# PASSIONLab/BELLA

Hardware: AMD Instinct MI355X
Metric: candidate overlap pairs/sec (higher is better)
Workload: dtype u16/u32 integer

## Files before the change

### bella_amd/csrc/bella_hip.hip

```cpp
#include <hip/hip_runtime.h>
#include <hipcub/hipcub.hpp>

#include <algorithm>
#include <cmath>
#include <initializer_list>
#include <iterator>
#include <map>
#include <cstdarg>
#include <cstdio>
#include <cstdlib>
#include <chrono>
#include <cstring>
#include <string>
#include <thread>
#include <vector>

#include "../../include/bella_hip.h"
#include "assemble.hpp"
#include "comm.hpp"
#include "core.hpp"
#include "fastq.hpp"
#include "kcount.hpp"
#include "logan.hpp"
#include "order.hpp"
// ... 80 lines not shown
    __host__ __device__ uint32_t operator()(const uint8_t& v) const { return (uint32_t)v; }
};
struct CountU64 {
    __host__ __device__ uint64_t operator()(const uint32_t& v) const { return (uint64_t)(v & ~kOrderedBit); }
};

}

struct bella_ctx {
    int device = 0;
    hipStream_t stream = nullptr;
    std::string err;
    uint32_t debug = 0;

    uint32_t nreads = 0;
    uint64_t total_bases = 0;
    Buf packed, roff;
    uint32_t nkmers = 0, kmer_size = 0;
    uint64_t nnz = 0;
    bool have_reads = false, have_matrix = false, have_pairs = false, have_alns = false;
    std::vector<std::string> names;
    std::vector<uint32_t> host_lens;
    bool have_tuples = false;
    uint64_t kc_ntuples = 0;
    uint32_t kc_nkmers = 0, kc_k = 0;
    uint32_t kc_bfirst = 0, kc_brows = 0;
    Buf kc_nk, kc_koff, kc_hist, kc_keys, kc_alt, kc_runlen, kc_flag, kc_slot, kc_nruns, kc_dcode, kc_dcount, kc_hkey, kc_hval, kc_found,
        kc_tstart, kc_cursor, kc_sel, kc_ringo, kc_ringp, kc_opos, kc_oid, kc_opos2, kc_oid2;
    Buf Bptr, Bk, Bpos, Bent, rowF, Aent, Aent2, Aov, Arow, Bloc;
    bool have_rowlists = false;
    bool want_rowlists = false;
    uint32_t part_first = 0, part_stride = 1;
    uint32_t layout_first = 0, layout_stride = 1;
    uint64_t owned_nnz = 0;
    uint64_t live_nnz = 0;
    uint64_t sym_sig[6] = {};
    uint64_t layout_gen = 0;
    uint32_t range_lo = 0, range_hi = 0xFFFFFFFFu;
    bool have_panel = false;
    uint32_t panel_first = 0, panel_rows = 0;
    uint64_t panel_nnz = 0;
    Buf t_kmer, t_read, t_pos, tstart, Bk_tmp, Bpos_tmp, rowcnt, asm_ws, asm_cls;
    Buf lk_key, lk_key2, lk_val, lk_val2, w, wscan, lk_rinfo;
    uint64_t flops = 0, npairs = 0;
    uint32_t pair_ratio1024 = 1024;
    bool long_list_sample = false;
#ifdef BELLA_DEV_PROF
    Buf prof;
#endif
    Buf flopsr, flopptr, nnzC, colptrC, rowlists, tiercaps, tmp_pairs, tmp_ext, pairs, ext, sortscr, ws,
        status, cubtmp, plist_hv, overflow, ctl, retry, orderlist, order_ws;
    bool order_attr = false;
    Buf w_f, w_off, w_key, w_key2, w_idx, w_idx2, w_hv, w_ovfl, w_plist, w_scr, w_rlen, w_rstart, w_rrank, w_redo, w_segfirst,
        w_toff, w_table, w_nruns, w_desc, w_gtab, w_gcount, w_gbase, w_rfirst, w_aent2, w_aov;
    uint32_t n_wide = 0;
    uint32_t n_retry = 0;
    uint32_t n_overflow = 0;
    uint64_t nalns = 0;
    Buf alns, seeds, xest, xest2, xids, xorder, xres, xstate, xlive, lg_res, lg_redo, lg_scratch;
    bool have_traces = false;
    std::vector<bella_trace> traces;
    std::vector<uint32_t> trace_ops;
    std::vector<uint32_t> batch_ops;
    bool have_batch_ops = false;
    bella_trace_stats trace_stats{};
    Buf tr_exts, tr_lists, tr_res, tr_pres, tr_opoff, tr_dirs, tr_scr, tr_ops;
    bella_timings tm{};
    hipEvent_t ev[12]{};
    uint32_t* pinned = nullptr;
    Stager stager;
    bella_ingest_stats ingest{};
    int caps_state = 0;
    ncclComm_t comm = nullptr;
    const Rccl* api = nullptr;
    int comm_ranks = 0, comm_rank = 0;
    Buf comm_meta;
    bool pass_known = false;
    uint64_t pass_sig[6] = {};
    uint32_t pass_tcnt[20] = {};
    uint64_t pass_products = 0;
    uint64_t pass_wide_products[2] = {};
    bool pass_rare_free = false;
    bool pass_big_free = false;
    uint32_t tier_caps[kNumTiers] = {};
    uint32_t ntiers = 0;
    bool tiers_from_env = false;
    uint64_t kcount_budget = 1ull << 30, wide_budget = 1ull << 30;
    bool lane_order_ok = true;
    uint64_t xdrop_class_min = 4ull * 4096 * 64;
    BufPool pool;
    uint32_t layout_inline = 0;
    uint32_t tune_layout_order = 0;
    uint32_t tune_inline = 0;
    uint32_t tune_row_path = 0;
    uint32_t tune_compact_b = 0;
    uint32_t tune_dist_layout = 2;
    bool dist_agreed = false;
    bool layout_dist = false;
    uint64_t tune_cache_bytes = 192ull << 20;
    uint32_t xdrop_variant = 1;
    size_t lds_attr[24] = {};
    hipStream_t side[kNumTiers + 1]{};
    hipEvent_t fork = nullptr, join[kNumTiers + 1]{};
};

namespace {

int fail(bella_ctx* c, int code, const char* fmt, ...) {
    char b[512];
    va_list ap;
    va_start(ap, fmt);
    vsnprintf(b, sizeof(b), fmt, ap);
    va_end(ap);
    if (c) c->err = b;
    return code;
}

#define HIPCHK(c, call)                                                                                           \
    do {                                                                                                          \
        hipError_t e_ = (call);                                                                                   \
        if (e_ != hipSuccess)                                                                                     \
            return fail(c, BELLA_ERR_HIP, "%s failed: %s (%s:%d)", #call, hipGetErrorString(e_), __FILE__, __LINE__); \
    } while (0)
#define KCHK(c) HIPCHK(c, hipGetLastError())
#define NCCLCHK(c, call)                                                                                          \
    do {                                                                                                          \
        ncclResult_t r_ = (call);                                                                                 \
        if (r_ != ncclSuccess)                                                                                    \
            return fail(c, BELLA_ERR_HIP, "%s failed: %s", #call, c->api && c->api->GetErrorString ? c->api->GetErrorString(r_) : "RCCL error"); \
    } while (0)

void release(Buf& b);
void trim_pool(BufPool& pl) {
    for (auto& q : pl.free) (void)hipFree(q.first);
    pl.free.clear();
    pl.bytes = 0;
}
int ensure_bytes(bella_ctx* c, Buf& b, size_t bytes) {
    if (bytes == 0) bytes = 16;
    if (b.cap >= bytes) return 0;
    release(b);
    BufPool& pl = c->pool;
    b.pool = &pl;
    const size_t want = bytes + bytes / 16 + 256;
    int best = -1;
    for (int i = 0; i < (int)pl.free.size(); ++i)
        if (pl.free[i].second >= want && pl.free[i].second <= 2 * want + (64ull << 20) && (best < 0 || pl.free[i].second < pl.free[best].second)) best = i;
    if (best >= 0) {
        b.p = pl.free[best].first; b.cap = pl.free[best].second;
        pl.bytes -= b.cap;
        pl.free.erase(pl.free.begin() + best);
        return 0;
    }
    if (pl.arena.base) {
        void* q = pl.arena.take(want);
        if (q) { b.p = q; b.cap = Arena::round(want); return 0; }
    }
    hipError_t e = hipMalloc(&b.p, want);
    if (e != hipSuccess && !pl.free.empty()) {
        (void)hipGetLastError();
        trim_pool(pl);
        e = hipMalloc(&b.p, want);
    }
    if (e != hipSuccess) {
        b.p = nullptr;
        return fail(c, BELLA_ERR_NOMEM, "hipMalloc(%zu) failed: %s", want, hipGetErrorString(e));
// ... 292 lines not shown
    uint32_t st = 0;
    int rc = read_status(c, &st);
    if (rc) return rc;
    rc = status_to_error(c, st);
    if (rc) return rc;
    c->pair_ratio1024 = ratio1024;
    release(c->lk_key); release(c->lk_key2); release(c->lk_val); release(c->lk_val2); release(c->w); release(c->wscan); release(c->lk_rinfo);
    c->tm.layout_ms = ev_ms(c->ev[4], c->ev[5]);
    c->have_matrix = true;
    c->layout_gen++;
    c->have_pairs = c->have_alns = false;
    return 0;
}

int check_params(bella_ctx* c, const bella_params* p) {
    if (!p) return fail(c, BELLA_ERR_BAD_ARG, "params is NULL");
    if (p->kmer_size != c->kmer_size)
        return fail(c, BELLA_ERR_BAD_ARG, "params.kmer_size (%u) differs from the matrix's (%u)", p->kmer_size, c->kmer_size);
    if (!p->skip_alignment) {
        if (p->xdrop > 127) return fail(c, BELLA_ERR_BAD_ARG, "params.xdrop must fit Xavier's int8 scores (<= 127)");
        if (!(p->error_rate >= 0.0 && p->error_rate <= 1.0) || !(p->delta_chernoff >= 0.0 && p->delta_chernoff <= 1.0))
            return fail(c, BELLA_ERR_BAD_ARG, "params.error_rate and params.delta_chernoff must lie in [0, 1]");
    }
    return 0;
}

}

extern "C" {

int bella_hip_abi_version(void) { return BELLA_HIP_ABI_VERSION; }

int bella_hip_device_count(void) {
    int n = 0;
    if (hipGetDeviceCount(&n) != hipSuccess) return 0;
    return n;
}

const char* bella_hip_strerror(int code) {
    switch (code) {
        case BELLA_OK: return "ok";
        case BELLA_ERR_NO_DEVICE: return "no gfx950 HIP device";
        case BELLA_ERR_HIP: return "HIP runtime error";
        case BELLA_ERR_BAD_ARG: return "bad argument";
        case BELLA_ERR_BAD_BASE: return "read contains a character other than ACGT";
        case BELLA_ERR_READ_TOO_LONG: return "read too long for 16-bit positions";
        case BELLA_ERR_TUPLE_ORDER: return "tuples not grouped by read";
        case BELLA_ERR_STATE: return "call order violated";
        case BELLA_ERR_ROW_TOO_LARGE: return "output column too large";
        case BELLA_ERR_BINS: return "more than 16 overlap bins";
        case BELLA_ERR_NOMEM: return "out of device memory";
    }
    return "unknown error";
}

const char* bella_hip_last_error(const bella_ctx* ctx) { return ctx ? ctx->err.c_str() : "null context"; }

int bella_hip_init(int device, bella_ctx** out) {
    if (!out) return BELLA_ERR_BAD_ARG;
    *out = nullptr;
    int n = 0;
    if (hipGetDeviceCount(&n) != hipSuccess || n <= 0 || device < 0 || device >= n) return BELLA_ERR_NO_DEVICE;
    hipDeviceProp_t prop;
    if (hipGetDeviceProperties(&prop, device) != hipSuccess) return BELLA_ERR_NO_DEVICE;
    if (std::strncmp(prop.gcnArchName, "gfx950", 6) != 0) return BELLA_ERR_NO_DEVICE;
    bella_ctx* c = new bella_ctx();
    c->device = device;
    c->ntiers = 0;
    for (uint32_t t = 0; t < kNumTiers; ++t) { c->tier_caps[t] = kTierCapsDefault[t]; c->ntiers = t + 1; if (kTierCapsDefault[t] == 65535) break; }
    hipError_t he = hipSetDevice(device);
    if (he == hipSuccess) he = hipStreamCreate(&c->stream);
    for (auto& e : c->ev) if (he == hipSuccess) he = hipEventCreate(&e);
    {
        int least = 0, greatest = 0;
        if (he == hipSuccess) he = hipDeviceGetStreamPriorityRange(&least, &greatest);
        int si = 0;
        for (auto& st : c->side) {
            if (he == hipSuccess) he = hipStreamCreateWithPriority(&st, hipStreamNonBlocking, si < 2 || si == kNumTiers ? greatest : least);
            ++si;
        }
    }
    if (he == hipSuccess) he = hipEventCreateWithFlags(&c->fork, hipEventDisableTiming);
    for (auto& e : c->join) if (he == hipSuccess) he = hipEventCreateWithFlags(&e, hipEventDisableTiming);
    if (he != hipSuccess) { bella_hip_destroy(c); return BELLA_ERR_HIP; }
    if (hipHostMalloc((void**)&c->pinned, 512, hipHostMallocDefault) != hipSuccess) { delete c; return BELLA_ERR_NOMEM; }
    if (ensure_bytes(c, c->status, 256)) { delete c; return BELLA_ERR_NOMEM; }
    (void)hipMemset(c->status.p, 0, 256);
    {
        uint32_t bad = 1;
        k_lane_order_selftest<<<1, 64, 0, c->stream>>>(ptr<uint32_t>(c->status) + 12);
        if (hipMemcpyAsync(&bad, ptr<uint32_t>(c->status) + 12, 4, hipMemcpyDeviceToHost, c->stream) != hipSuccess ||
            hipStreamSynchronize(c->stream) != hipSuccess) bad = 1;
        c->lane_order_ok = bad == 0;
        c->tm.lane_order = c->lane_order_ok ? 1u : 2u;
    }
    *out = c;
    return 0;
}

void bella_hip_destroy(bella_ctx* c) {
    if (!c) return;
    (void)hipSetDevice(c->device);
    (void)hipStreamSynchronize(c->stream);
    if (c->comm && c->api) { (void)c->api->CommDestroy(c->comm); c->comm = nullptr; }
    release(c->comm_meta);
    Buf* all[] = {&c->packed, &c->roff, &c->Bptr, &c->Bk, &c->Bpos, &c->Bent, &c->rowF, &c->Aent, &c->Aent2, &c->Aov, &c->Arow, &c->Bloc, &c->t_kmer, &c->t_read, &c->t_pos,
                  &c->tstart, &c->Bk_tmp, &c->Bpos_tmp, &c->rowcnt, &c->asm_ws, &c->asm_cls, &c->lk_key, &c->lk_key2, &c->lk_val, &c->lk_val2, &c->lk_rinfo,
                  &c->w, &c->wscan, &c->flopsr, &c->flopptr, &c->nnzC, &c->colptrC,
                  &c->rowlists, &c->tiercaps, &c->tmp_pairs, &c->tmp_ext, &c->pairs, &c->ext, &c->sortscr, &c->ws,
                  &c->status, &c->cubtmp, &c->alns, &c->seeds, &c->plist_hv, &c->overflow, &c->ctl, &c->retry, &c->orderlist, &c->order_ws, &c->w_f, &c->w_off, &c->w_key, &c->w_key2, &c->w_idx, &c->w_idx2, &c->w_hv, &c->w_ovfl,
                  &c->w_plist, &c->w_scr, &c->w_rlen, &c->w_rstart, &c->w_rrank, &c->w_redo, &c->w_segfirst, &c->w_toff, &c->w_table, &c->w_nruns, &c->w_desc, &c->w_gtab, &c->w_gcount, &c->w_gbase, &c->w_rfirst, &c->w_aent2, &c->w_aov, &c->kc_nk, &c->kc_koff, &c->kc_hist, &c->kc_keys, &c->kc_alt, &c->kc_runlen,
                  &c->kc_flag, &c->kc_slot, &c->kc_nruns, &c->kc_dcode, &c->kc_dcount, &c->kc_hkey, &c->kc_hval, &c->kc_found, &c->kc_tstart, &c->kc_cursor, &c->kc_sel, &c->kc_ringo, &c->kc_ringp, &c->kc_opos, &c->kc_oid, &c->kc_opos2, &c->kc_oid2, &c->xest, &c->xest2, &c->xids, &c->xorder, &c->xres, &c->xstate, &c->xlive, &c->lg_res, &c->lg_redo, &c->lg_scratch};
    for (Buf* b : all) release(*b);
    trim_pool(c->pool);
    if (c->pool.arena.base) { (void)hipFree(c->pool.arena.base); c->pool.arena = Arena(); }
    for (auto& e : c->ev) (void)hipEventDestroy(e);
    for (auto& st : c->side) (void)hipStreamDestroy(st);
    (void)hipEventDestroy(c->fork);
    for (auto& e : c->join) (void)hipEventDestroy(e);
    (void)hipStreamDestroy(c->stream);
    if (c->pinned) (void)hipHostFree(c->pinned);
    c->stager.destroy();
    delete c;
}

int bella_hip_set_tuning(bella_ctx* c, uint32_t what, const uint64_t* values, uint32_t n) {
    if (!c || (n && !values)) return BELLA_ERR_BAD_ARG;
    switch (what) {
        case BELLA_TUNE_LDS_TIERS: {
            uint32_t caps[kNumTiers];
            uint32_t m = 0;
            for (uint32_t q = 0; q < n && m + 1 < kNumTiers; ++q) {
                const uint64_t v = values[q];
                if (v < 64 || v > 11008 || (m && v <= caps[m - 1])) return fail(c, BELLA_ERR_BAD_ARG, "tier caps must ascend within [64, 11008]");
                caps[m++] = (uint32_t)v;
            }
            if (m) {
                for (uint32_t t = 0; t < m; ++t) c->tier_caps[t] = caps[t];
                c->tier_caps[m] = 65535;
                c->ntiers = m + 1;
                c->tiers_from_env = true;
            } else {
                c->ntiers = 0;
                for (uint32_t t = 0; t < kNumTiers; ++t) { c->tier_caps[t] = kTierCapsDefault[t]; c->ntiers = t + 1; if (kTierCapsDefault[t] == 65535) break; }
                c->tiers_from_env = false;
            }
            c->caps_state = 0;
            c->pass_known = false;
            return 0;
        }
        case BELLA_TUNE_KCOUNT_BUDGET: c->kcount_budget = n && values[0] ? values[0] : (1ull << 30); return 0;
        case BELLA_TUNE_WIDE_BUDGET: c->wide_budget = n && values[0] ? values[0] : (1ull << 30); return 0;
        case BELLA_TUNE_XDROP_VARIANT:
            if (n && values[0] > 3) return fail(c, BELLA_ERR_BAD_ARG, "x-drop variant 0..3");
            c->xdrop_variant = n ? (uint32_t)values[0] : 1u;
            return 0;
        case BELLA_TUNE_XDROP_CLASS_MIN: c->xdrop_class_min = n ? values[0] : 4ull * 4096 * 64; return 0;
        case BELLA_TUNE_ROW_LISTS:
            if (n && values[0] > 1) return fail(c, BELLA_ERR_BAD_ARG, "row lists: 0 or 1");
            c->want_rowlists = n && values[0] == 1;
            return 0;
        case BELLA_TUNE_LAYOUT_ORDER:
            if (n && values[0] > 1) return fail(c, BELLA_ERR_BAD_ARG, "layout order: 0 (k-mer order) or 1 (first appearance)");
            c->tune_layout_order = n ? (uint32_t)values[0] : 0u;
            return 0;
        case BELLA_TUNE_INLINE_ENTRIES:
// ... 1885 lines not shown
        if (main_l >= 0) { rc = side_stream(2); if (rc) return rc; sst = c->side[2]; }
        a.rowdesc = ptr<uint4>(c->rowlists) + (size_t)(g_ntiers - 1) * nr;
        a.nrows = tcnt[g_ntiers - 1];
        a.cap = tier_caps[g_ntiers - 1];
        a.dcap = a.cap;
        const unsigned grid = a.nrows < kGlobalGrid ? a.nrows : kGlobalGrid;
        if (c->have_rowlists) k_spgemm_rows_global<true><<<grid, kGlobalBlock, 0, sst>>>(a);
        else k_spgemm_rows_global<false><<<grid, kGlobalBlock, 0, sst>>>(a);
        KCHK(c);
        launches++;
    }
    {
        int side_left = 3 - nwhole - (global_tier ? 1 : 0);
        for (int l = nl - 1; l >= 0; --l) {
            if (!ln[l].rows || (whole_cu(l) && l != main_l)) continue;
            int later = 0;
            for (int m2 = 0; m2 < l; ++m2) later += ln[m2].rows ? 1 : 0;
            const bool on_main = l == main_l || side_left == 0 || later == 0;
            if (!on_main) side_left--;
            rc = launch_class(l, on_main);
            if (rc) return rc;
        }
    }
    if (c->n_wide) {
        hipStream_t const main_stream = c->stream, wst = c->side[kNumTiers];
        c->stream = wst;
        int rw = 0;
        if (wide_begun) rw = wide_batch_finish(c, wide_batch, false);
        else {
            HIPCHK(c, hipStreamWaitEvent(wst, c->ev[3], 0));
            rw = wide_columns();
            if (!rw) rw = run_wide(c, a, c->n_wide, widelist, wide_products);
        }
        c->stream = main_stream;
        if (rw) { (void)hipStreamSynchronize(wst); return rw; }
        HIPCHK(c, hipEventRecord(c->join[kNumTiers], wst));
        HIPCHK(c, hipStreamWaitEvent(c->stream, c->join[kNumTiers], 0));
    }
    for (int w = 0; w < 3; ++w)
        if (used[w]) {
            HIPCHK(c, hipEventRecord(c->join[w], c->side[w]));
            HIPCHK(c, hipStreamWaitEvent(c->stream, c->join[w], 0));
        }
    FoldArgs fa;
    fa.ctl = a.ctl;
    fa.overflow = a.overflow;
    fa.flopptr = a.flopptr;
    fa.plist = a.plist;
    fa.roff = a.roff;
    fa.packed = a.packed;
    fa.tmp_pairs = a.tmp_pairs;
    fa.tmp_ext = a.tmp_ext;
    fa.sort_scratch = ptr<uint16_t>(c->sortscr);
    fa.k = a.k;
    fa.binSize = a.binSize;
    auto rerun_columns = [&]() -> int {
        a.rowlist = ptr<uint32_t>(c->retry);
        a.rowdesc = nullptr;
        a.nrows_dev = ptr<uint32_t>(c->ctl) + kCtlRetry;
        if (c->have_rowlists) k_spgemm_rows_global<true><<<kRerunGrid, kGlobalBlock, 0, c->stream>>>(a);
        else k_spgemm_rows_global<false><<<kRerunGrid, kGlobalBlock, 0, c->stream>>>(a);
        KCHK(c);
        return 0;
    };
    auto finish = [&]() -> int {
        if ((uint64_t)nr + 1 <= kScanSingleMax) {
            k_scan_counts<<<1, 1024, 0, c->stream>>>(ptr<uint32_t>(c->nnzC), ptr<uint64_t>(c->colptrC), nr + 1);
            KCHK(c);
        } else {
            hipcub::TransformInputIterator<uint64_t, CountU64, const uint32_t*> it(ptr<uint32_t>(c->nnzC), CountU64());
            size_t tb = c->cubtmp.cap;
            HIPCHK(c, hipcub::DeviceScan::ExclusiveSum(c->cubtmp.p, tb, it, ptr<uint64_t>(c->colptrC), (int)nr + 1, c->stream));
        }
        EVREC(6);
        if (nr) {
            OrderArgs oa;
            oa.flopptr = ptr<uint64_t>(c->flopptr); oa.colptrC = ptr<uint64_t>(c->colptrC); oa.nnzC = ptr<uint32_t>(c->nnzC);
            oa.flops = ptr<uint32_t>(c->flopsr);
            oa.nreads = nr; oa.i0 = i0; oa.stride = c->part_stride; oa.nown = nown;
            oa.tmp_pairs = ptr<bella_pair>(c->tmp_pairs); oa.tmp_ext = want_ext ? ptr<bella_pair_ext>(c->tmp_ext) : nullptr;
            oa.pairs = ptr<bella_pair>(c->pairs); oa.ext = want_ext ? ptr<bella_pair_ext>(c->ext) : nullptr;
            oa.totals = (uint64_t*)(d_ctl + kCtlTotals);
            oa.nbig = d_ctl + kCtlOrderBig; oa.biglist = ptr<uint32_t>(c->orderlist); oa.ws = ptr<uint8_t>(c->order_ws);
            if (nown <= kOrderOneLaunchMax) {
                k_order_wave<kOrderWaveHt, 0><<<nblk(nown ? nown : 1, kOrderBlock / 64), kOrderBlock, 0, c->stream>>>(oa);
                KCHK(c);
            } else {
                k_order_wave<512, 0><<<nblk(nown ? nown : 1, kOrderBlock / 64), kOrderBlock, 0, c->stream>>>(oa);
                KCHK(c);
                k_order_wave<kOrderWaveHt, 512><<<nblk(nown ? nown : 1, kOrderBlock / 64), kOrderBlock, 0, c->stream>>>(oa);
                KCHK(c);
            }
            if (!skip_big) {
                k_order_block<<<kOrderBigGrid, kOrderBlock, (size_t)6 * kOrderLdsHt, c->stream>>>(oa);
                KCHK(c);
            }
        }
        EVREC(7);
        HIPCHK(c, hipMemcpyAsync(ctl_host, d_ctl, 4 * kCtlWords, hipMemcpyDeviceToHost, c->stream));
        return 0;
    };
    if (!skip_rare) { rc = rerun_columns(); if (rc) return rc; }
    EVREC(5);
    if (!skip_rare) { k_fold_overflow<<<256, 64, 0, c->stream>>>(fa); KCHK(c); EVREC(8); }
    return finish();
    };
#undef EVREC
    rc = enqueue();
    if (rc) return rc;
    HIPCHK(c, hipStreamSynchronize(c->stream));
    if ((skip_rare && (ctl_host[kCtlRetry] || ctl_host[kCtlOverflow])) || (skip_big && ctl_host[kCtlOrderBig])) {
        c->pass_rare_free = false;
        c->pass_big_free = false;
        if (depth > 0) return fail(c, BELLA_ERR_STATE, "internal: rare kernels still skipped");
        return run_spgemm(c, p, status_out, depth + 1);
    }
    const uint32_t* const tcnt = c->pass_tcnt;
    const uint64_t Fub = c->pass_products;
    uint64_t P = 0, F = 0;
    std::memcpy(&P, ctl_host + kCtlTotals, 8);
    std::memcpy(&F, ctl_host + kCtlTotals + 2, 8);
    rc = status_to_error(c, ctl_host[kCtlStatus] & ~1u);
    if (rc) return rc;
    *status_out = ctl_host[kCtlStatus];
    c->n_overflow = ctl_host[kCtlOverflow];
    c->n_retry = ctl_host[kCtlRetry];
    c->npairs = P;
    c->flops = F;
    if (F != Fub || std::memcmp(ctl_host + kCtlTierCnt, tcnt, 4 * (g_ntiers + 1)) != 0) {
        c->pass_known = false;
        return fail(c, BELLA_ERR_STATE, "internal: product total %llu / tier lengths differ from the ones the pass was sized with (%llu)",
                    (unsigned long long)F, (unsigned long long)Fub);
    }
    c->pass_known = true;
    c->pass_rare_free = c->n_retry == 0 && c->n_overflow == 0 && c->n_wide == 0;
    c->pass_big_free = ctl_host[kCtlOrderBig] == 0;
    c->tm.symbolic_ms = ev_ms(c->ev[2], c->ev[3]);
    c->tm.spgemm_ms = ev_ms(c->ev[3], c->ev[5]);
    c->tm.fold_ms = skip_rare ? 0.f : ev_ms(c->ev[5], c->ev[8]);
    c->tm.compact_ms = ev_ms(c->ev[6], c->ev[7]);
    c->tm.overlap_total_ms = ev_ms(c->ev[2], c->ev[7]);
    c->tm.spgemm_launches = launches;
    c->tm.retry_columns = c->n_retry;
    c->tm.overflow_pairs = c->n_overflow;
#ifdef BELLA_DEV_PROF
    {
        unsigned long long ph[10 * kNumTiers];
        HIPCHK(c, hipMemcpy(ph, c->prof.p, sizeof(ph), hipMemcpyDeviceToHost));
        static const char* nm[9] = {"expand", "gather+insert", "count-scan", "scatter+singles", "rank/overlay", "parents", "walks", "emit", "head (descriptor + first entries + table init)"};
        for (int l = 0; l < nl; ++l) {
            const unsigned long long* q = ph + 10 * l;
            if (!q[9]) continue;
            double tot = 1e-9;
            for (int n = 0; n < 9; ++n) tot += (double)q[n];
            fprintf(stderr, "[bella_hip prof] class cap %u (%llu columns, %.0f cycles each):", tier_caps[ln[l].hi], q[9], tot / (double)q[9]);
            for (int n = 0; n < 9; ++n) fprintf(stderr, " %s %.1f%%", nm[n], 100.0 * (double)q[n] / tot);
            fprintf(stderr, "\n");
        }
    }
#endif
    return 0;
}

static uint32_t owned_columns(const bella_ctx* c, uint32_t* i0_out) {
    const uint32_t nr = c->nreads;
    const uint32_t hi = c->range_hi < nr ? c->range_hi : nr;
    uint32_t i0 = c->range_lo + (c->part_first + c->part_stride - c->range_lo % c->part_stride) % c->part_stride;
    const uint32_t nown = i0 < hi ? (hi - i0 + c->part_stride - 1) / c->part_stride : 0;
    if (!nown) i0 = 0;
    if (i0_out) *i0_out = i0;
    return nown;
}

int bella_hip_overlap(bella_ctx* c, const bella_params* p, uint64_t* npairs, uint64_t* flops) {
    if (!c) return BELLA_ERR_BAD_ARG;
// ... 778 lines not shown
```

### bella_amd/csrc/order.hpp

```cpp
#pragma once
#include <hip/hip_runtime.h>
#include <stdint.h>
#include "../../include/bella_hip.h"
#include "core.hpp"
#include "slotorder.hpp"
#include "util.hpp"

namespace bella {

constexpr uint32_t kOrderWaveHt = 1024;
constexpr uint32_t kOrderLdsHt = 16384;
constexpr uint32_t kOrderBlock = 256;
constexpr uint32_t kOrderBigGrid = 512;
constexpr uint32_t kOrderOneLaunchMax = 32768;
constexpr uint64_t kOrderWsBytes = (uint64_t)6 * 65536;

struct OrderArgs {
    const uint64_t* flopptr;
    const uint64_t* colptrC;
    const uint32_t* nnzC;
    const uint32_t* flops;
    uint32_t nreads, i0, stride, nown;
    const bella_pair* tmp_pairs;
    const bella_pair_ext* tmp_ext;
    bella_pair* pairs;
    bella_pair_ext* ext;
    uint64_t* totals;
    uint32_t* nbig;
    uint32_t* biglist;
    uint8_t* ws;
};

__device__ __forceinline__ void order_copy_record(const OrderArgs& a, uint64_t from, uint64_t to, uint32_t cid) {
    uint4 rec = *(const uint4*)(a.tmp_pairs + from);
    asm volatile("" : "+v"(rec.y));
    rec.y = cid;
    *(uint4*)(a.pairs + to) = rec;
    if (a.ext) a.ext[to] = a.tmp_ext[from];
}

__device__ __forceinline__ bool wave_next_free(const uint32_t* T2, uint16_t* nf, uint32_t ht) {
    const uint32_t lane = lane_id();
    const uint32_t nb = (ht + 63u) >> 6;
    uint32_t carry = 0xFFFFFFFFu;
#pragma unroll 1
    for (int sweep = 0; sweep < 2; ++sweep) {
        for (uint32_t b = nb; b-- > 0;) {
            const uint32_t s = (b << 6) + lane;
            const bool empty = s < ht && T2[s] == kEmpty;
            const unsigned long long m = __ballot(empty);
            if (sweep == 1 && s < ht) {
                const unsigned long long up = m >> lane;
                nf[s] = (uint16_t)(up ? s + (uint32_t)__ffsll((long long)up) - 1u : carry);
            }
            if (m) carry = (b << 6) + (uint32_t)__ffsll((long long)m) - 1u;
        }
        if (carry == 0xFFFFFFFFu) return false;
    }
    return true;
}
__device__ __forceinline__ void wave_rank_slots(const uint32_t* T2, uint16_t* ord, uint32_t ht) {
    const uint32_t lane = lane_id();
    const uint32_t nb = (ht + 63u) >> 6;
    uint32_t base = 0;
    for (uint32_t b = 0; b < nb; ++b) {
        const uint32_t s = (b << 6) + lane;
        const uint32_t it = s < ht ? T2[s] : kEmpty;
        const unsigned long long m = __ballot(it != kEmpty);
        if (it != kEmpty) ord[base + (uint32_t)__popcll(m & ((1ull << lane) - 1ull))] = (uint16_t)(it & 0xFFFFu);
        base += (uint32_t)__popcll(m);
    }
}

template <uint32_t HT, uint32_t HTLO>
__global__ __launch_bounds__(kOrderBlock) void k_order_wave(OrderArgs a) {
    __shared__ uint32_t s_T2[kOrderBlock / 64][HT];
    __shared__ uint16_t s_ord[kOrderBlock / 64][HT];
    const uint32_t j0 = blockIdx.x * (kOrderBlock / 64) + wave_id();
    const uint32_t lane = lane_id();
    if (HTLO == 0 && j0 == 0 && lane == 0) a.totals[0] = a.colptrC[a.nreads];
    if (j0 >= a.nown) return;
    const uint32_t i = a.i0 + j0 * a.stride;
    uint32_t nz = a.nnzC[i];
    uint64_t src = a.flopptr[i], dst = a.colptrC[i];
    uint32_t tmax = a.flops[i];
    asm volatile("" : "+v"(nz), "+v"(src), "+v"(dst), "+v"(tmax));
    const uint32_t d = nz & ~kOrderedBit;
    if (!d) return;
    if (nz & kOrderedBit) {
        if (HTLO == 0) for (uint32_t r = lane; r < d; r += 64) order_copy_record(a, src + r, dst + r, i);
        return;
    }
    const uint32_t ht = pow2_at_least(16u, d);
    if (ht > kOrderWaveHt) {
        if (HTLO == 0 && lane == 0) a.biglist[atomicAdd(a.nbig, 1u)] = i;
        return;
    }
    if (ht > HT || ht <= HTLO) return;
    uint32_t* T2 = s_T2[wave_id()];
    uint16_t* ord = s_ord[wave_id()];
    for (uint32_t s = lane; s < ht; s += 64) T2[s] = kEmpty;
    constexpr uint32_t NI = HT / 64;
    uint32_t key[NI], fp[NI];
#pragma unroll
    for (uint32_t u = 0; u < NI; ++u) {
        const uint32_t j = lane + 64 * u;
        key[u] = 0; fp[u] = 0xFFFFFFFFu;
        if (j < d) { const uint2 kf = *(const uint2*)(a.tmp_pairs + src + j); key[u] = kf.x; fp[u] = kf.y; }
    }
    group_sync<64>();
    uint32_t prev = 0;
    for (uint32_t rd = 0;; ++rd) {
        const uint32_t bound = round_bound(rd, ht, d, tmax);
        if (rd) { (void)wave_next_free(T2, ord, ht); group_sync<64>(); }
#pragma unroll
        for (uint32_t u = 0; u < NI; ++u) {
            if (fp[u] < prev || fp[u] >= bound) continue;
            const uint32_t home = (key[u] * 107u) & (ht - 1), item = (fp[u] << 16) | (lane + 64 * u);
            if (rd) slot_insert<true>(T2, ord, ht - 1, home, item);
            else slot_insert<false>(T2, ord, ht - 1, home, item);
        }
        group_sync<64>();
        if (bound >= tmax) break;
        prev = bound;
    }
    wave_rank_slots(T2, ord, ht);
    group_sync<64>();
    {
        uint32_t r = lane;
        for (; r + 192 < d; r += 256) {
            uint4 rec[4];
#pragma unroll
            for (uint32_t u = 0; u < 4; ++u) rec[u] = *(const uint4*)(a.tmp_pairs + src + ord[r + 64 * u]);
#pragma unroll
            for (uint32_t u = 0; u < 4; ++u) { asm volatile("" : "+v"(rec[u].y)); rec[u].y = i; *(uint4*)(a.pairs + dst + r + 64 * u) = rec[u]; }
            if (a.ext) {
#pragma unroll
                for (uint32_t u = 0; u < 4; ++u) a.ext[dst + r + 64 * u] = a.tmp_ext[src + ord[r + 64 * u]];
            }
        }
        for (; r < d; r += 64) order_copy_record(a, src + ord[r], dst + r, i);
    }
}

__global__ __launch_bounds__(kOrderBlock) void k_order_block(OrderArgs a) {
    extern __shared__ __attribute__((aligned(16))) uint8_t smem[];
    __shared__ uint32_t scr[16];
    const uint32_t nbig = *a.nbig;
    const uint32_t tid = threadIdx.x;
    for (uint32_t x = blockIdx.x; x < nbig; x += gridDim.x) {
        const uint32_t i = a.biglist[x];
        const uint32_t d = a.nnzC[i] & ~kOrderedBit;
        const uint64_t src = a.flopptr[i], dst = a.colptrC[i];
        const uint32_t ht = pow2_at_least(16u, d);
        uint32_t* T2;
        uint16_t* ord;
        if (ht <= kOrderLdsHt) { T2 = (uint32_t*)smem; ord = (uint16_t*)(smem + (size_t)4 * kOrderLdsHt); }
        else { uint8_t* w = a.ws + (uint64_t)blockIdx.x * kOrderWsBytes; T2 = (uint32_t*)w; ord = (uint16_t*)(w + (size_t)4 * 65536); }
        for (uint32_t s = tid; s < ht; s += kOrderBlock) T2[s] = kEmpty;
        __syncthreads();
        const uint32_t tmax = a.flops[i];
        uint32_t prev = 0;
        for (uint32_t rd = 0;; ++rd) {
            const uint32_t bound = round_bound(rd, ht, d, tmax);
            if (rd) { (void)build_next_free<(int)kOrderBlock>(T2, ord, ht, scr); __syncthreads(); }
            for (uint32_t j = tid; j < d; j += kOrderBlock) {
                const uint2 kf = *(const uint2*)(a.tmp_pairs + src + j);
                if (kf.y < prev || kf.y >= bound) continue;
                const uint32_t home = (kf.x * 107u) & (ht - 1), item = (kf.y << 16) | j;
                if (rd) slot_insert<true>(T2, ord, ht - 1, home, item);
                else slot_insert<false>(T2, ord, ht - 1, home, item);
            }
            __syncthreads();
            if (bound >= tmax) break;
            prev = bound;
        }
        {
            const uint32_t c = (ht + kOrderBlock - 1) / kOrderBlock;
            const uint32_t lo = tid * c < ht ? tid * c : ht, hi = lo + c < ht ? lo + c : ht;
            uint32_t occ = 0;
            for (uint32_t s = lo; s < hi; ++s) occ += T2[s] != kEmpty ? 1u : 0u;
            uint32_t tot;
            uint32_t rank = block_excl_scan<kOrderBlock / 64>(occ, scr, &tot);
            for (uint32_t s = lo; s < hi; ++s) {
                const uint32_t it = T2[s];
                if (it != kEmpty) ord[rank++] = (uint16_t)(it & 0xFFFFu);
            }
        }
        __syncthreads();
        for (uint32_t r = tid; r < d; r += kOrderBlock) order_copy_record(a, src + ord[r], dst + r, i);
        __syncthreads();
    }
}

}
```

### bella_amd/csrc/spgemm.hpp

```cpp
#pragma once
#include <hip/hip_runtime.h>
#include <type_traits>
#include "../../include/bella_hip.h"
#include "core.hpp"
#include "util.hpp"

namespace bella {

constexpr uint32_t kSU = 4;
constexpr uint32_t kScatterChunk = 64;
#ifndef BELLA_WALK_W
#define BELLA_WALK_W 8
#endif
#ifndef BELLA_GATHER_BATCH
#define BELLA_GATHER_BATCH(blk) 2u
#endif
#ifndef BELLA_SCATTER_CHUNKS
#define BELLA_SCATTER_CHUNKS 8
#endif
#ifndef BELLA_SCATTER_WAVES
#define BELLA_SCATTER_WAVES 1
#endif
#ifndef BELLA_WALK_W_GLOBAL
#define BELLA_WALK_W_GLOBAL 32
#endif
#ifndef BELLA_ROW_BLOCK
#define BELLA_ROW_BLOCK 512
#endif
constexpr int kRowBlock = BELLA_ROW_BLOCK;
constexpr uint32_t kCtlOverflow = 17;
constexpr uint32_t kCtlWork2 = 18;
constexpr uint32_t kCtlStatus = 19;
constexpr uint32_t kCtlRetry = 21;
constexpr uint32_t kCtlOrderBig = 22;
constexpr uint32_t kCtlTierCnt = 32;
constexpr uint32_t kCtlTotals = 48;
constexpr uint32_t kCtlWords = 64;

struct SpgemmArgs {
    const uint32_t* rowlist;
    const uint4* rowdesc;
    uint32_t nrows;
    uint32_t tier_lo, tier_hi;
    uint32_t tcount[4];
    uint32_t tcount_valid;
    uint32_t nreads;
    const uint32_t* Bptr;
    const uint2* Bent;
    uint32_t inl;
    const uint2* Aent;
    const uint2* Aent2;
    const uint16_t* Aov;
    const uint64_t* Arow;
    const uint64_t* roff;
    const uint32_t* packed;
    const uint64_t* flopptr;
    const uint32_t* flops;
    bella_pair* tmp_pairs;
    bella_pair_ext* tmp_ext;
    uint32_t* nnzC;
    uint2* plist;
    uint4* overflow;
    uint32_t* ctl;
    uint32_t* retry;
    const uint32_t* nrows_dev;
    uint8_t* ws;
    uint64_t ws_stride;
    uint32_t cap;
    uint32_t dcap;
    int k;
    int binSize;
#ifdef BELLA_DEV_PROF
    unsigned long long* prof;
    int stop_phase;
#endif
    int inject_unordered;
};

constexpr uint32_t kRowScratchBytes = 256;
__host__ __device__ inline size_t row_mem_bytes(uint32_t cap, uint32_t dcap, bool overlay) {
    return kRowScratchBytes + (size_t)8 * cap + (size_t)16 * dcap + (overlay ? 2 : 4) * (size_t)((cap + 3) & ~3u) + 2 * (size_t)((dcap + 1) & ~1u) +
           (overlay ? 0 : (size_t)8 * cap + 2 * (size_t)((cap + 3) & ~3u));
}

struct RowMem {
    uint32_t* scr;
    uint32_t* A_hv;
    uint32_t* A_gov;
    uint32_t* T1key;
    uint32_t* T1cnt;
    uint32_t* T1first;
    uint32_t* Gaux;
    uint16_t* S_p;
    uint32_t* M;
    uint8_t* A_fl;
    uint8_t* L_fl;
    uint32_t* L_hv;
    uint32_t* L_gov;
    uint32_t cap, dcap;
};

__device__ __forceinline__ RowMem carve(uint8_t* base, uint32_t cap, uint32_t dcap, bool overlay) {
    RowMem m;
    m.scr = (uint32_t*)base;
    uint32_t* w = (uint32_t*)(base + kRowScratchBytes);
    m.A_hv = w;            w += cap;
    m.A_gov = w;           w += cap;
    m.T1key = w;           w += dcap;
    m.T1cnt = w;           w += dcap;
    m.T1first = w;         w += dcap;
    m.Gaux = w;            w += dcap;
    m.S_p = (uint16_t*)w;  w += (overlay ? 1 : 2) * (((cap + 3) & ~3u) / 2);
    m.M = w;               w += (dcap + 1) / 2;
    if (overlay) { m.L_hv = m.A_hv; m.L_gov = m.A_gov; m.A_fl = nullptr; m.L_fl = nullptr; }
    else { m.L_hv = w; w += cap; m.L_gov = w; w += cap; m.A_fl = (uint8_t*)w; w += (cap + 3) / 4; m.L_fl = (uint8_t*)w; }
    m.cap = cap;
    m.dcap = dcap;
// ... 814 lines not shown
```

Measured before the change: 12.77 billion.

## Make order kernel persistent with ticketed column batches and software prefetch

Replaces the one-wave-per-column order kernel (with its two-launch split by hash table size) with a persistent kernel sized from occupancy. Waves pull batches of columns through an atomic ticket counter and prefetch the next column's descriptor and key/fingerprint data while the current column is processed, using per-lane loads reduced with readlane. Small and large hash tables are dispatched inside one kernel by template NI. This is meant to cut launch and tail imbalance and hide load latency, at the cost of extra register pressure (prefetch arrays of 16 entries) and an atomic per batch; the ticket counter must be zeroed before each launch.

```diff
diff --git a/bella_amd/csrc/bella_hip.hip b/bella_amd/csrc/bella_hip.hip
--- a/bella_amd/csrc/bella_hip.hip
+++ b/bella_amd/csrc/bella_hip.hip
@@ -186,6 +186,7 @@
     uint64_t pass_wide_products[2] = {};
     bool pass_rare_free = false;
     bool pass_big_free = false;
+    uint32_t order_blocks = 1;
     uint32_t tier_caps[kNumTiers] = {};
     uint32_t ntiers = 0;
     bool tiers_from_env = false;
@@ -644,6 +645,11 @@
     }
     if (he == hipSuccess) he = hipEventCreateWithFlags(&c->fork, hipEventDisableTiming);
     for (auto& e : c->join) if (he == hipSuccess) he = hipEventCreateWithFlags(&e, hipEventDisableTiming);
+    {
+        int per_cu = 0;
+        if (he == hipSuccess) he = hipOccupancyMaxActiveBlocksPerMultiprocessor(&per_cu, k_order_wave, (int)kOrderBlock, 0);
+        if (he == hipSuccess && per_cu > 0) c->order_blocks = (uint32_t)per_cu * (uint32_t)prop.multiProcessorCount;
+    }
     if (he != hipSuccess) { bella_hip_destroy(c); return BELLA_ERR_HIP; }
     if (hipHostMalloc((void**)&c->pinned, 512, hipHostMallocDefault) != hipSuccess) { delete c; return BELLA_ERR_NOMEM; }
     if (ensure_bytes(c, c->status, 256)) { delete c; return BELLA_ERR_NOMEM; }
@@ -2695,15 +2701,9 @@
             oa.pairs = ptr<bella_pair>(c->pairs); oa.ext = want_ext ? ptr<bella_pair_ext>(c->ext) : nullptr;
             oa.totals = (uint64_t*)(d_ctl + kCtlTotals);
             oa.nbig = d_ctl + kCtlOrderBig; oa.biglist = ptr<uint32_t>(c->orderlist); oa.ws = ptr<uint8_t>(c->order_ws);
-            if (nown <= kOrderOneLaunchMax) {
-                k_order_wave<kOrderWaveHt, 0><<<nblk(nown ? nown : 1, kOrderBlock / 64), kOrderBlock, 0, c->stream>>>(oa);
-                KCHK(c);
-            } else {
-                k_order_wave<512, 0><<<nblk(nown ? nown : 1, kOrderBlock / 64), kOrderBlock, 0, c->stream>>>(oa);
-                KCHK(c);
-                k_order_wave<kOrderWaveHt, 512><<<nblk(nown ? nown : 1, kOrderBlock / 64), kOrderBlock, 0, c->stream>>>(oa);
-                KCHK(c);
-            }
+            oa.ticket = d_ctl + kCtlOrderTicket;
+            k_order_wave<<<std::min(c->order_blocks, nblk(nown ? nown : 1, kOrderBlock / 64)), kOrderBlock, 0, c->stream>>>(oa);
+            KCHK(c);
             if (!skip_big) {
                 k_order_block<<<kOrderBigGrid, kOrderBlock, (size_t)6 * kOrderLdsHt, c->stream>>>(oa);
                 KCHK(c);
diff --git a/bella_amd/csrc/order.hpp b/bella_amd/csrc/order.hpp
--- a/bella_amd/csrc/order.hpp
+++ b/bella_amd/csrc/order.hpp
@@ -12,7 +12,8 @@
 constexpr uint32_t kOrderLdsHt = 16384;
 constexpr uint32_t kOrderBlock = 256;
 constexpr uint32_t kOrderBigGrid = 512;
-constexpr uint32_t kOrderOneLaunchMax = 32768;
+constexpr uint32_t kOrderSmallHt = 512;
+constexpr uint32_t kOrderBatch = 4;
 constexpr uint64_t kOrderWsBytes = (uint64_t)6 * 65536;
 
 struct OrderArgs {
@@ -27,6 +28,7 @@
     bella_pair_ext* ext;
     uint64_t* totals;
     uint32_t* nbig;
+    uint32_t* ticket;
     uint32_t* biglist;
     uint8_t* ws;
 };
@@ -72,42 +74,72 @@
     }
 }
 
-template <uint32_t HT, uint32_t HTLO>
-__global__ __launch_bounds__(kOrderBlock) void k_order_wave(OrderArgs a) {
-    __shared__ uint32_t s_T2[kOrderBlock / 64][HT];
-    __shared__ uint16_t s_ord[kOrderBlock / 64][HT];
-    const uint32_t j0 = blockIdx.x * (kOrderBlock / 64) + wave_id();
-    const uint32_t lane = lane_id();
-    if (HTLO == 0 && j0 == 0 && lane == 0) a.totals[0] = a.colptrC[a.nreads];
-    if (j0 >= a.nown) return;
-    const uint32_t i = a.i0 + j0 * a.stride;
-    uint32_t nz = a.nnzC[i];
-    uint64_t src = a.flopptr[i], dst = a.colptrC[i];
-    uint32_t tmax = a.flops[i];
-    asm volatile("" : "+v"(nz), "+v"(src), "+v"(dst), "+v"(tmax));
-    const uint32_t d = nz & ~kOrderedBit;
-    if (!d) return;
-    if (nz & kOrderedBit) {
-        if (HTLO == 0) for (uint32_t r = lane; r < d; r += 64) order_copy_record(a, src + r, dst + r, i);
-        return;
-    }
-    const uint32_t ht = pow2_at_least(16u, d);
-    if (ht > kOrderWaveHt) {
-        if (HTLO == 0 && lane == 0) a.biglist[atomicAdd(a.nbig, 1u)] = i;
-        return;
-    }
-    if (ht > HT || ht <= HTLO) return;
-    uint32_t* T2 = s_T2[wave_id()];
-    uint16_t* ord = s_ord[wave_id()];
+enum : uint32_t { kOrdNone = 0, kOrdSmall = 1, kOrdLarge = 2, kOrdCopy = 3, kOrdBig = 4 };
+struct OrderDesc { uint32_t w; };
+struct OrderCol {
+    uint32_t i, d, ht, tmax, kind;
+    uint64_t src, dst;
+};
+
+__device__ __forceinline__ uint32_t uniform_(uint32_t v) { return (uint32_t)__builtin_amdgcn_readfirstlane((int)v); }
+
+__device__ __forceinline__ uint32_t lane_opaque() {
+    uint32_t lane = lane_id();
+    asm volatile("" : "+v"(lane));
+    return lane;
+}
+__device__ __forceinline__ void order_desc_issue(const OrderArgs& a, uint32_t t, OrderDesc& D) {
+    D.w = 0;
+    if (t < a.nown) {
+        const uint32_t i = a.i0 + t * a.stride, lane = lane_opaque();
+        const uint32_t* p = lane == 0 ? a.nnzC + i : lane == 1 ? a.flops + i : lane < 4 ? (const uint32_t*)(a.flopptr + i) + (lane - 2)
+                                                                                      : (const uint32_t*)(a.colptrC + i) + (lane - 4);
+        if (lane < 6) D.w = *p;
+    }
+}
+__device__ __forceinline__ void order_desc_take(const OrderArgs& a, uint32_t t, const OrderDesc& D, OrderCol& C) {
+    const uint32_t nz = (uint32_t)__builtin_amdgcn_readlane((int)D.w, 0);
+    C.i = a.i0 + t * a.stride;
+    C.d = nz & ~kOrderedBit;
+    C.tmax = (uint32_t)__builtin_amdgcn_readlane((int)D.w, 1);
+    C.src = (uint64_t)(uint32_t)__builtin_amdgcn_readlane((int)D.w, 2) | ((uint64_t)(uint32_t)__builtin_amdgcn_readlane((int)D.w, 3) << 32);
+    C.dst = (uint64_t)(uint32_t)__builtin_amdgcn_readlane((int)D.w, 4) | ((uint64_t)(uint32_t)__builtin_amdgcn_readlane((int)D.w, 5) << 32);
+    C.ht = pow2_at_least(16u, C.d <= kOrderWaveHt ? C.d : 0u);
+    C.kind = t >= a.nown || !C.d ? kOrdNone : (nz & kOrderedBit) ? kOrdCopy : C.d > kOrderWaveHt ? kOrdBig : C.ht <= kOrderSmallHt ? kOrdSmall : kOrdLarge;
+}
+struct OrderTickets { uint32_t base, k, inflight; bool on; };
+__device__ __forceinline__ uint32_t order_ticket_issue(const OrderArgs& a, bool on) {
+    uint32_t t = 0;
+    if (on && lane_id() == 0) t = atomicAdd(a.ticket, 1u);
+    return t;
+}
+__device__ __forceinline__ uint32_t order_next_column(const OrderArgs& a, uint32_t G, OrderTickets& T) {
+    if (++T.k >= kOrderBatch) {
+        T.base = T.on ? G + uniform_(T.inflight) * kOrderBatch : a.nown;
+        T.k = 0;
+        T.inflight = order_ticket_issue(a, T.on);
+    }
+    return T.base + T.k;
+}
+
+__device__ __forceinline__ void order_kf_issue(const OrderArgs& a, const OrderCol& C, uint2 (&pre)[16]) {
+    const uint32_t lane = lane_opaque();
+    const uint32_t n = C.kind == kOrdSmall || C.kind == kOrdLarge ? C.d : 0u;
+#pragma unroll
+    for (uint32_t u = 0; u < 16; ++u) {
+        const char* const base = (const char*)(a.tmp_pairs + C.src + 64 * u);
+        pre[u] = make_uint2(0u, 0u);
+        if (lane + 64 * u < n) pre[u] = *(const uint2*)(base + lane * 16u);
+    }
+}
+__device__ __forceinline__ void order_kf_pack(const OrderCol& C, const uint2 (&pre)[16], uint32_t (&cur)[16]) {
+#pragma unroll
+    for (uint32_t u = 0; u < 16; ++u) cur[u] = (((pre[u].x * 107u) & (C.ht - 1)) << 16) | (pre[u].y & 0xFFFFu);
+}
+template <uint32_t NI>
+__device__ __forceinline__ void order_insert_rank(const OrderCol& C, const uint32_t (&cur)[16], uint32_t* T2, uint16_t* ord) {
+    const uint32_t lane = lane_opaque(), ht = C.ht, d = C.d, tmax = C.tmax;
     for (uint32_t s = lane; s < ht; s += 64) T2[s] = kEmpty;
-    constexpr uint32_t NI = HT / 64;
-    uint32_t key[NI], fp[NI];
-#pragma unroll
-    for (uint32_t u = 0; u < NI; ++u) {
-        const uint32_t j = lane + 64 * u;
-        key[u] = 0; fp[u] = 0xFFFFFFFFu;
-        if (j < d) { const uint2 kf = *(const uint2*)(a.tmp_pairs + src + j); key[u] = kf.x; fp[u] = kf.y; }
-    }
     group_sync<64>();
     uint32_t prev = 0;
     for (uint32_t rd = 0;; ++rd) {
@@ -115,8 +147,11 @@
         if (rd) { (void)wave_next_free(T2, ord, ht); group_sync<64>(); }
 #pragma unroll
         for (uint32_t u = 0; u < NI; ++u) {
-            if (fp[u] < prev || fp[u] >= bound) continue;
-            const uint32_t home = (key[u] * 107u) & (ht - 1), item = (fp[u] << 16) | (lane + 64 * u);
+            uint32_t cv = cur[u];
+            asm volatile("" : "+v"(cv));
+            const uint32_t fp = cv & 0xFFFFu;
+            if (lane + 64 * u >= d || fp < prev || fp >= bound) continue;
+            const uint32_t home = cv >> 16, item = (fp << 16) | (lane + 64 * u);
             if (rd) slot_insert<true>(T2, ord, ht - 1, home, item);
             else slot_insert<false>(T2, ord, ht - 1, home, item);
         }
@@ -126,20 +161,67 @@
     }
     wave_rank_slots(T2, ord, ht);
     group_sync<64>();
-    {
-        uint32_t r = lane;
-        for (; r + 192 < d; r += 256) {
-            uint4 rec[4];
-#pragma unroll
-            for (uint32_t u = 0; u < 4; ++u) rec[u] = *(const uint4*)(a.tmp_pairs + src + ord[r + 64 * u]);
-#pragma unroll
-            for (uint32_t u = 0; u < 4; ++u) { asm volatile("" : "+v"(rec[u].y)); rec[u].y = i; *(uint4*)(a.pairs + dst + r + 64 * u) = rec[u]; }
-            if (a.ext) {
-#pragma unroll
-                for (uint32_t u = 0; u < 4; ++u) a.ext[dst + r + 64 * u] = a.tmp_ext[src + ord[r + 64 * u]];
-            }
-        }
-        for (; r < d; r += 64) order_copy_record(a, src + ord[r], dst + r, i);
+}
+__device__ __forceinline__ void order_move(const OrderArgs& a, const OrderCol& C, const uint16_t* ord) {
+    const uint32_t lane = lane_opaque(), d = C.d;
+    const char* const from = (const char*)(a.tmp_pairs + C.src);
+    char* const to = (char*)(a.pairs + C.dst);
+    uint32_t r = lane;
+    for (; r + 192 < d; r += 256) {
+        uint4 rec[4];
+#pragma unroll
+        for (uint32_t u = 0; u < 4; ++u) rec[u] = *(const uint4*)(from + (uint32_t)ord[r + 64 * u] * 16u);
+#pragma unroll
+        for (uint32_t u = 0; u < 4; ++u) { asm volatile("" : "+v"(rec[u].y)); rec[u].y = C.i; *(uint4*)(to + (r + 64 * u) * 16u) = rec[u]; }
+        if (a.ext) {
+#pragma unroll
+            for (uint32_t u = 0; u < 4; ++u) a.ext[C.dst + r + 64 * u] = a.tmp_ext[C.src + ord[r + 64 * u]];
+        }
+    }
+    for (; r < d; r += 64) order_copy_record(a, C.src + ord[r], C.dst + r, C.i);
+}
+
+__global__ __launch_bounds__(kOrderBlock, 5) void k_order_wave(OrderArgs a) {
+    __shared__ uint32_t s_T2[kOrderBlock / 64][kOrderWaveHt];
+    __shared__ uint16_t s_ord[kOrderBlock / 64][kOrderWaveHt];
+    uint32_t* const T2 = s_T2[wave_id()];
+    uint16_t* const ord = s_ord[wave_id()];
+    const uint32_t lane = lane_id();
+    const uint32_t G = gridDim.x * (kOrderBlock / 64);
+    const uint32_t w = uniform_(blockIdx.x * (kOrderBlock / 64) + wave_id());
+    if (w == 0 && lane == 0) a.totals[0] = a.colptrC[a.nreads];
+    if (w >= a.nown) return;
+
+    OrderCol C, N, NN;
+    OrderDesc D;
+    uint32_t tC = w, tN, tD;
+    OrderTickets T;
+    uint2 pre[16];
+    uint32_t cur[16];
+    T.on = G < a.nown; T.base = 0; T.k = kOrderBatch;
+    order_desc_issue(a, tC, D);
+    T.inflight = order_ticket_issue(a, T.on);
+    order_desc_take(a, tC, D, C);
+    order_kf_issue(a, C, pre);
+    tN = order_next_column(a, G, T);
+    order_desc_issue(a, tN, D);
+    order_kf_pack(C, pre, cur);
+    order_desc_take(a, tN, D, N);
+    order_kf_issue(a, N, pre);
+    tD = order_next_column(a, G, T);
+    order_desc_issue(a, tD, D);
+    while (tC < a.nown) {
+        if (C.kind == kOrdSmall) { order_insert_rank<8>(C, cur, T2, ord); order_move(a, C, ord); }
+        else if (C.kind == kOrdLarge) { order_insert_rank<16>(C, cur, T2, ord); order_move(a, C, ord); }
+        else if (C.kind == kOrdCopy) { for (uint32_t r = lane; r < C.d; r += 64) order_copy_record(a, C.src + r, C.dst + r, C.i); }
+        else if (C.kind == kOrdBig) { if (lane == 0) a.biglist[atomicAdd(a.nbig, 1u)] = C.i; }
+        order_kf_pack(N, pre, cur);
+        order_desc_take(a, tD, D, NN);
+        C = N; N = NN;
+        tC = tN; tN = tD;
+        order_kf_issue(a, N, pre);
+        tD = order_next_column(a, G, T);
+        order_desc_issue(a, tD, D);
     }
 }
 
diff --git a/bella_amd/csrc/spgemm.hpp b/bella_amd/csrc/spgemm.hpp
--- a/bella_amd/csrc/spgemm.hpp
+++ b/bella_amd/csrc/spgemm.hpp
@@ -33,6 +33,7 @@
 constexpr uint32_t kCtlStatus = 19;
 constexpr uint32_t kCtlRetry = 21;
 constexpr uint32_t kCtlOrderBig = 22;
+constexpr uint32_t kCtlOrderTicket = 23;
 constexpr uint32_t kCtlTierCnt = 32;
 constexpr uint32_t kCtlTotals = 48;
 constexpr uint32_t kCtlWords = 64;
```

Result: slower. 12.37 billion (-3.1%).
